# dusk-network/plonk

Hardware: NVIDIA H100
Metric: proofs/sec @ 2^16 gates (higher is better)
Workload: dtype u32 limbs (Fr 256-bit / Fp 384-bit Montgomery)

## Files before the change

### plonk_b200/csrc/msm.cu

```cuda
#include <algorithm>
#include <atomic>
#include <vector>

#include "common.cuh"
#include "g1.cuh"
#include "host_field.h"

struct pb200_srs {
  size_t n_points;
  int c;
  int W;
  uint4* table;
};

namespace pb {

static constexpr int kGroup = 8;
static constexpr unsigned kClassChunk = 512;
static constexpr unsigned kHeavyMin = 32, kHeavyFactor = 4;
static constexpr unsigned kHeavyChunk = 256;

PB_D G1Affine ld_affine(const uint4* p, size_t i) {
  const uint4* q = p + 6 * i;
  uint4 a0 = __ldg(q), a1 = __ldg(q + 1), a2 = __ldg(q + 2), b0 = __ldg(q + 3), b1 = __ldg(q + 4), b2 = __ldg(q + 5);
  G1Affine r;
  r.x.v[0] = a0.x; r.x.v[1] = a0.y; r.x.v[2] = a0.z; r.x.v[3] = a0.w;
  r.x.v[4] = a1.x; r.x.v[5] = a1.y; r.x.v[6] = a1.z; r.x.v[7] = a1.w;
  r.x.v[8] = a2.x; r.x.v[9] = a2.y; r.x.v[10] = a2.z; r.x.v[11] = a2.w;
  r.y.v[0] = b0.x; r.y.v[1] = b0.y; r.y.v[2] = b0.z; r.y.v[3] = b0.w;
  r.y.v[4] = b1.x; r.y.v[5] = b1.y; r.y.v[6] = b1.z; r.y.v[7] = b1.w;
  r.y.v[8] = b2.x; r.y.v[9] = b2.y; r.y.v[10] = b2.z; r.y.v[11] = b2.w;
  return r;
}
PB_D void st_fp(uint4* q, const Fp& f) {
  q[0] = make_uint4(f.v[0], f.v[1], f.v[2], f.v[3]);
  q[1] = make_uint4(f.v[4], f.v[5], f.v[6], f.v[7]);
  q[2] = make_uint4(f.v[8], f.v[9], f.v[10], f.v[11]);
}
PB_D Fp ld_fp(const uint4* q) {
  uint4 a = q[0], b = q[1], c = q[2];
  Fp f;
  f.v[0] = a.x; f.v[1] = a.y; f.v[2] = a.z; f.v[3] = a.w;
  f.v[4] = b.x; f.v[5] = b.y; f.v[6] = b.z; f.v[7] = b.w;
// ... 181 lines not shown
      val &= mask;
    }
    unsigned d = val + carry;
    unsigned sign = 0;
    if (d > half) {
      d = (1u << c) - d;
      sign = 1;
      carry = 1;
    } else {
      carry = 0;
    }
    const size_t slot = ((size_t)b * W + w) * n + i;
    if (d == 0) {
      ebkt[slot] = 0xffffffffu;
    } else {
      const unsigned bucket = d - 1;
      ebkt[slot] = (bucket << 1) | sign;
      epos[slot] = atomicAdd(&counts[(size_t)b * nb + bucket], 1u);
    }
  }
}

__global__ void __launch_bounds__(1024) k_msm_scan(const unsigned* counts, unsigned* offsets, unsigned* order, unsigned* n_heavy,
                                                   unsigned* heavy_pre, unsigned* max_len, unsigned nb, int size_shift) {
  __shared__ unsigned sums[1024];
  __shared__ unsigned bins[1024];
  __shared__ unsigned s_nh, s_total, s_thr_units, s_max;
  const unsigned b = blockIdx.x, tid = threadIdx.x;
  const unsigned* cnt = counts + (size_t)b * nb;
  unsigned* off = offsets + (size_t)b * (nb + 1);
  unsigned* ord = order + (size_t)b * nb;
  const unsigned chunk = (nb + 1023) / 1024;
  const unsigned lo = tid * chunk, hi = min(nb, lo + chunk);
  unsigned s = 0, mx = 0;
  for (unsigned k = lo; k < hi; k++) {
    s += cnt[k];
    mx = max(mx, cnt[k]);
  }
  sums[tid] = s;
  bins[tid] = 0;
  if (tid == 0) s_max = 0;
  __syncthreads();
  if (mx) atomicMax(&s_max, mx);
  for (unsigned d = 1; d < 1024; d <<= 1) {
    unsigned v = (tid >= d) ? sums[tid - d] : 0;
    __syncthreads();
    sums[tid] += v;
// ... 22 lines not shown
  }
  bins[tid] = sums[tid] - mine;
  if (tid == 0) {
    const unsigned avg = s_total / nb;
    const unsigned thr = max(kHeavyMin, kHeavyFactor * avg);
    s_thr_units = min(1021u, (thr + (1u << size_shift) - 1u) >> size_shift);
  }
  __syncthreads();
  if (tid == 1022u - s_thr_units) {
    n_heavy[b] = sums[tid];
    s_nh = sums[tid];
  }
  __syncthreads();
  for (unsigned k = tid; k < nb; k += 1024) {
    const unsigned pos = atomicAdd(&bins[1023u - min(cnt[k] >> size_shift, 1023u)], 1u);
    ord[pos] = k;
  }
  __syncthreads();
  const unsigned nh = s_nh;
  unsigned* hp = heavy_pre + (size_t)b * (nb + 1);
  const unsigned per = (nh + 1023u) / 1024u;
  const unsigned h_lo = min(nh, tid * per), h_hi = min(nh, h_lo + per);
  unsigned c = 0;
  for (unsigned h = h_lo; h < h_hi; h++) c += (cnt[ord[h]] + kHeavyChunk - 1) / kHeavyChunk;
  sums[tid] = c;
  __syncthreads();
  for (unsigned d = 1; d < 1024; d <<= 1) {
    unsigned v = (tid >= d) ? sums[tid - d] : 0;
    __syncthreads();
    sums[tid] += v;
    __syncthreads();
  }
  unsigned run2 = sums[tid] - c;
  for (unsigned h = h_lo; h < h_hi; h++) {
    hp[h] = run2;
    run2 += (cnt[ord[h]] + kHeavyChunk - 1) / kHeavyChunk;
  }
  if (tid == 1023) hp[nh] = sums[1023];
}

__global__ void k_msm_scatter(const unsigned* ebkt, const unsigned* epos, const unsigned* offsets, size_t n,
                              int W, unsigned nb, size_t n_table, size_t first, unsigned* sorted) {
  size_t i = (size_t)blockIdx.x * blockDim.x + threadIdx.x;
  if (i >= n) return;
  const unsigned w = blockIdx.y, b = blockIdx.z;
  const size_t slot = ((size_t)b * W + w) * n + i;
  const unsigned e = ebkt[slot];
  if (e == 0xffffffffu) return;
  const unsigned bucket = e >> 1, sign = e & 1u;
  const unsigned dst = offsets[(size_t)b * (nb + 1) + bucket] + epos[slot];
  sorted[(size_t)b * n * W + dst] = (unsigned)(((size_t)w * n_table + first + i) << 1) | sign;
}

PB_D G1Xyzz shfl_down_xyzz(const G1Xyzz& p, int delta, int width) {
  G1Xyzz r;
#pragma unroll
  for (int i = 0; i < 12; i++) {
    r.x.v[i] = __shfl_down_sync(0xffffffffu, p.x.v[i], delta, width);
    r.y.v[i] = __shfl_down_sync(0xffffffffu, p.y.v[i], delta, width);
// ... 38 lines not shown
      p_next = ld_affine(table, e_next >> 1);
    }
    if (p.is_inf()) continue;
    if (e & 1u) p.y = p.y.neg();
    xyzz_madd(acc, p.x, p.y);
  }
  for (int d = (int)split >> 1; d > 0; d >>= 1) {
    G1Xyzz o = shfl_down_xyzz(acc, d, (int)split);
    xyzz_add(acc, o);
  }
  if (valid && part == 0) st_xyzz(sums, (size_t)b * nb + bucket, acc);
}

PB_D G1Xyzz warp_sum(G1Xyzz v) {
  for (int d = 16; d > 0; d >>= 1) {
    G1Xyzz o = shfl_down_xyzz(v, d, 32);
    xyzz_add(v, o);
  }
  return v;
}

__global__ void __launch_bounds__(128) k_msm_heavy_chunks(const uint4* table, const unsigned* sorted, const unsigned* offsets,
                                                          const unsigned* order, const unsigned* n_heavy, const unsigned* heavy_pre,
                                                          unsigned nb, size_t cap, size_t part_cap, uint4* partials) {
  const unsigned b = blockIdx.y;
  const unsigned nh = n_heavy[b];
  if (nh == 0) return;
  const unsigned* hp = heavy_pre + (size_t)b * (nb + 1);
  const unsigned total = hp[nh];
  const unsigned* src = sorted + (size_t)b * cap;
  const unsigned* off = offsets + (size_t)b * (nb + 1);
  const unsigned* ord = order + (size_t)b * nb;
  const unsigned lane = threadIdx.x & 31, warps = gridDim.x * 4;
  for (unsigned v = blockIdx.x * 4 + (threadIdx.x >> 5); v < total; v += warps) {
    unsigned lo = 0, hi = nh;
    while (hi - lo > 1) {
      const unsigned mid = (lo + hi) >> 1;
      if (hp[mid] <= v) lo = mid; else hi = mid;
    }
    const unsigned bucket = ord[lo];
    const unsigned start = off[bucket] + (v - hp[lo]) * kHeavyChunk, end = min(off[bucket + 1], start + kHeavyChunk);
    G1Xyzz acc = G1Xyzz::identity();
    for (unsigned k = start + lane; k < end; k += 32) {
      const unsigned e = __ldg(src + k);
      G1Affine p = ld_affine(table, e >> 1);
      if (p.is_inf()) continue;
      if (e & 1u) p.y = p.y.neg();
      xyzz_madd(acc, p.x, p.y);
    }
    acc = warp_sum(acc);
    if (lane == 0) st_xyzz(partials, (size_t)b * part_cap + v, acc);
  }
}

__global__ void __launch_bounds__(128) k_msm_heavy_combine(const uint4* partials, const unsigned* order, const unsigned* n_heavy,
                                                           const unsigned* heavy_pre, unsigned nb, size_t part_cap, uint4* sums) {
  const unsigned b = blockIdx.y;
  const unsigned nh = n_heavy[b];
  const unsigned* hp = heavy_pre + (size_t)b * (nb + 1);
  const unsigned lane = threadIdx.x & 31, warps = gridDim.x * 4;
  for (unsigned h = blockIdx.x * 4 + (threadIdx.x >> 5); h < nh; h += warps) {
    G1Xyzz acc = G1Xyzz::identity();
    for (unsigned v = hp[h] + lane; v < hp[h + 1]; v += 32) {
      G1Xyzz q = ld_xyzz(partials, (size_t)b * part_cap + v);
// ... 344 lines not shown
  fetch(np - 1);
  Fp inv_run = ld_fp(a.ctot + 3 * ((size_t)b * a.ctas_max + blockIdx.x)) * ld_fp(a.factor + 3 * ((size_t)b * a.threads + t));
#pragma unroll 1
  for (int i = np - 1; i >= 0; i--) {
    const uint4 ds = a.desc[slot0 + (size_t)i * a.threads];
    asm volatile("cp.async.wait_group 0;" ::: "memory");
    G1Affine p1, p2;
    p1.x = ld_fp(stage); p1.y = ld_fp(stage + 3);
    p2.x = ld_fp(stage + 6); p2.y = ld_fp(stage + 9);
    const Fp pre = ld_fp(stage + 12);
    if (i > 0) fetch(i - 1);
    if (FIRST) {
      if ((ds.x & 1u) && !p1.is_inf()) p1.y = p1.y.neg();
      if ((ds.y & 1u) && !p2.is_inf()) p2.y = p2.y.neg();
    }
    Fp d = Fp::one();
    const int kind = aff_classify(p1, p2, &d);
    const Fp inv_d = inv_run * pre;
    inv_run = inv_run * d;
    aff_store(a, b, ds.z, aff_finish(kind, p1, p2, inv_d));
  }
}

struct DigitPlan {
  int ndig;
  int shift[8];
  int bits[8];
  int first_class[8];
  int n_digit_classes;
  int n_a_classes;
  int nclasses;
};

template <bool AFFINE>
__global__ void __launch_bounds__(64) k_msm_groups(const uint4* sums, unsigned nb, int g, uint4* S, uint4* A) {
  const unsigned G = blockIdx.x * blockDim.x + threadIdx.x;
  const unsigned n_groups = nb / g;
  if (G >= n_groups) return;
  const unsigned b = blockIdx.y;
  G1Xyzz run = G1Xyzz::identity(), acc = G1Xyzz::identity();
  for (int j = g - 1; j >= 0; j--) {
    if (AFFINE) {
      const G1Affine q = ld_affine(sums, (size_t)b * nb + (size_t)G * g + j);
      if (!q.is_inf()) xyzz_madd(run, q.x, q.y);
    } else {
      G1Xyzz q = ld_xyzz(sums, (size_t)b * nb + (size_t)G * g + j);
      xyzz_add(run, q);
    }
    xyzz_add(acc, run);
  }
  st_xyzz(S, (size_t)b * n_groups + G, run);
  st_xyzz(A, (size_t)b * n_groups + G, acc);
}

__global__ void __launch_bounds__(128) k_msm_group_classes(const uint4* S, const uint4* A, unsigned n_groups,
                                                           DigitPlan plan, unsigned chunks, uint4* out) {
  const int cls = blockIdx.x * 4 + (threadIdx.x >> 5);
  const int lane = threadIdx.x & 31;
  const unsigned b = blockIdx.y, chunk = blockIdx.z;
  if (cls >= plan.nclasses) return;
  G1Xyzz acc = G1Xyzz::identity();
  if (cls < plan.n_digit_classes) {
    int j = 0;
    while (j + 1 < plan.ndig && cls >= plan.first_class[j + 1]) j++;
    const unsigned v = cls - plan.first_class[j];
    const int sh_j = plan.shift[j], bits_j = plan.bits[j];
    const unsigned count = n_groups >> bits_j;
    for (unsigned idx = chunk * kClassChunk + lane; idx < min(count, (chunk + 1) * kClassChunk); idx += 32) {
      const unsigned G = ((idx >> sh_j) << (sh_j + bits_j)) | (v << sh_j) | (idx & ((1u << sh_j) - 1u));
      G1Xyzz q = ld_xyzz(S, (size_t)b * n_groups + G);
      xyzz_add(acc, q);
    }
  } else if (chunk == 0) {
    const unsigned first = (unsigned)(cls - plan.n_digit_classes) * 256u;
    for (unsigned G = first + lane; G < min(n_groups, first + 256u); G += 32) {
      G1Xyzz q = ld_xyzz(A, (size_t)b * n_groups + G);
      xyzz_add(acc, q);
    }
  }
  acc = warp_sum(acc);
  if (lane == 0) st_xyzz(out, ((size_t)b * plan.nclasses + cls) * chunks + chunk, acc);
}

__global__ void __launch_bounds__(256) k_msm_final(const uint4* classes, DigitPlan plan, unsigned chunks, uint4* out) {
  const int lane = threadIdx.x & 31, j = threadIdx.x >> 5;
  const unsigned b = blockIdx.x;
  if (j < plan.ndig) {
    const int nv = 1 << plan.bits[j];
    G1Xyzz x = G1Xyzz::identity();
    if (lane < nv)
      for (unsigned ch = 0; ch < chunks; ch++) {
        G1Xyzz q = ld_xyzz(classes, ((size_t)b * plan.nclasses + plan.first_class[j] + lane) * chunks + ch);
        xyzz_add(x, q);
      }
    for (int d = 1; d < nv; d <<= 1) {
      G1Xyzz o = shfl_down_xyzz(x, d, 32);
      if (lane + d < nv) xyzz_add(x, o);
    }
    G1Xyzz y = (lane >= 1 && lane < nv) ? x : G1Xyzz::identity();
    for (int d = nv >> 1; d > 0; d >>= 1) {
      G1Xyzz o = shfl_down_xyzz(y, d, 32);
      xyzz_add(y, o);
    }
    if (lane == 0) st_xyzz(out, (size_t)b * (plan.ndig + 1) + j, y);
  } else if (j == 7) {
    G1Xyzz acc = G1Xyzz::identity();
    for (int k = lane; k < plan.n_a_classes; k += 32) {
      G1Xyzz q = ld_xyzz(classes, ((size_t)b * plan.nclasses + plan.n_digit_classes + k) * chunks);
      xyzz_add(acc, q);
    }
    acc = warp_sum(acc);
    if (lane == 0) st_xyzz(out, (size_t)b * (plan.ndig + 1) + plan.ndig, acc);
  }
}

__global__ void k_selftest_fr_mul(const uint4* a, const uint4* b, uint4* o, size_t n) {
  size_t i = (size_t)blockIdx.x * blockDim.x + threadIdx.x;
  if (i >= n) return;
  Fr x, y;
  uint4 t0 = a[2 * i], t1 = a[2 * i + 1];
  x.v[0] = t0.x; x.v[1] = t0.y; x.v[2] = t0.z; x.v[3] = t0.w; x.v[4] = t1.x; x.v[5] = t1.y; x.v[6] = t1.z; x.v[7] = t1.w;
  t0 = b[2 * i]; t1 = b[2 * i + 1];
  y.v[0] = t0.x; y.v[1] = t0.y; y.v[2] = t0.z; y.v[3] = t0.w; y.v[4] = t1.x; y.v[5] = t1.y; y.v[6] = t1.z; y.v[7] = t1.w;
  Fr r = x * y;
  o[2 * i] = make_uint4(r.v[0], r.v[1], r.v[2], r.v[3]);
  o[2 * i + 1] = make_uint4(r.v[4], r.v[5], r.v[6], r.v[7]);
}
__global__ void k_selftest_fp_mul(const uint4* a, const uint4* b, uint4* o, size_t n) {
  size_t i = (size_t)blockIdx.x * blockDim.x + threadIdx.x;
  if (i >= n) return;
  Fp x = ld_fp(a + 3 * i), y = ld_fp(b + 3 * i);
  st_fp(o + 3 * i, x * y);
}

__global__ void k_selftest_fp_ops(const uint4* a, const uint4* b, const uint4* c, const uint4* d, uint4* o, size_t n) {
  size_t i = (size_t)blockIdx.x * blockDim.x + threadIdx.x;
// ... 39 lines not shown
std::atomic<int> g_prof_on{0};
std::atomic<uint64_t> g_prof_acc_ns{0}, g_prof_acc_adds{0}, g_prof_acc_launches{0}, g_prof_acc_points{0};
std::atomic<uint64_t> g_prof_sp_ns{0}, g_prof_sp_adds{0}, g_prof_sp_launches{0}, g_prof_sp_points{0};

static int pick_window(size_t n_points) {
  if (const char* env = getenv("PB200_MSM_C")) {
    int c = atoi(env);
    if (c >= 2 && c <= 20) return c;
  }
  int lg = 0;
  while (((size_t)1 << (lg + 1)) <= n_points) lg++;
  if (lg <= 16) return std::max(4, lg);
  return lg <= 19 ? 16 : 20;
}

static void xyzz_dev_to_host(const uint32_t* w, pbh::HXyzz* o) {
  memcpy(o->x.v, w, 48);
  memcpy(o->y.v, w + 12, 48);
  memcpy(o->zz.v, w + 24, 48);
  memcpy(o->zzz.v, w + 36, 48);
}

thread_local int t_msm_throughput_hint = 0;

struct MsmTail {
  DigitPlan plan;
  int log_g = 0;
  int c = 0;
  uint32_t batch = 0;
  size_t words_per_entry() const { return (size_t)(plan.ndig + 1) * 48; }
};

static bool msm_affine_enabled() {
  static const bool on = [] {
    const char* e = getenv("PB200_MSM_AFFINE");
    return e && atoi(e) != 0;
  }();
  return on;
}

static size_t aff_slots(size_t cap, size_t nb) {
  size_t widest = 0;
  for (int r = 0; ((size_t)1 << r) < cap || r == 0; r++) {
    const size_t positions = r == 0 ? cap : (cap >> r) + nb + 1;
    const size_t ctas = ((positions + kAffK - 1) / kAffK + kAffThreads - 1) / kAffThreads;
    widest = std::max(widest, ctas * kAffThreads);
// ... 2 lines not shown
}

static int msm_plan_c(int c, uint32_t batch, MsmTail* tail, unsigned* n_groups_out, int* g_out) {
  const unsigned nb = 1u << (c - 1);
  const int g = std::min<unsigned>(kGroup, nb);
  const unsigned n_groups = nb / g;
  int log_g = 0;
  while ((1 << log_g) < g) log_g++;
  DigitPlan& plan = tail->plan;
  int total_bits = 0;
  while ((1u << total_bits) < n_groups) total_bits++;
  plan.ndig = (total_bits + 3) / 4;
  if (plan.ndig > 7) return fail(PB200_ERR_INVALID_ARG, "window too wide for the bucket reduction");
  int sh = 0, cls = 0;
  for (int j = 0; j < plan.ndig; j++) {
    const int bits = (total_bits - sh) / (plan.ndig - j);
    plan.shift[j] = sh;
    plan.bits[j] = bits;
    plan.first_class[j] = cls;
    sh += bits;
    cls += 1 << bits;
  }
  plan.n_digit_classes = cls;
  plan.n_a_classes = (int)((n_groups + 255) / 256);
  plan.nclasses = plan.n_digit_classes + plan.n_a_classes;
  tail->log_g = log_g;
  tail->c = c;
  tail->batch = batch;
  *n_groups_out = n_groups;
  *g_out = g;
  return 0;
}
static int msm_plan(const pb200_srs* srs, uint32_t batch, MsmTail* tail, unsigned* n_groups_out, int* g_out) {
  return msm_plan_c(srs->c, batch, tail, n_groups_out, g_out);
}

static int msm_enqueue(const pb200_srs* srs, size_t first, const uint64_t* d_scalars, size_t n, uint32_t batch, size_t stride,
                       cudaStream_t st, ScratchScope& scope, uint4** d_result, MsmTail* tail, cudaEvent_t* prof_ev,
                       const unsigned** d_totals) {
  if (first + n > srs->n_points) return fail(PB200_ERR_DEGREE_TOO_LARGE, "more scalars than commit-key points");
  const int c = srs->c, W = srs->W;
  const unsigned nb = 1u << (c - 1);
  const size_t cap = n * (size_t)W;
  if (((srs->n_points * (size_t)W) << 1) >= ((size_t)1 << 32)) return fail(PB200_ERR_INVALID_ARG, "commit key too large for 32-bit point references");
  unsigned n_groups = 0;
  int g = 0;
  PB_TRY(msm_plan(srs, batch, tail, &n_groups, &g));
  const DigitPlan& plan = tail->plan;
  uint4* result = nullptr;
  PB_ALLOC(scope, result, (size_t)batch * (plan.ndig + 1) * 192);
  *d_result = result;
  if (n == 0) {
    PB_CUDA(cudaMemsetAsync(result, 0, (size_t)batch * (plan.ndig + 1) * 192, st));
    return 0;
  }

  int log_split = 0;
  if (!t_msm_throughput_hint) {
    const size_t avg = cap / nb;
    while (log_split < 5 && ((size_t)nb * batch << log_split) < (1u << 17) && (avg >> (log_split + 1)) >= 8) log_split++;
  }
  if (const char* env = getenv("PB200_MSM_LOG_SPLIT")) log_split = atoi(env);

  unsigned *counts = nullptr, *offsets = nullptr, *order = nullptr, *ebkt = nullptr, *epos = nullptr, *sorted = nullptr;
  uint4 *sums = nullptr, *classes = nullptr, *S = nullptr, *A = nullptr;
  PB_ALLOC(scope, counts, (size_t)batch * nb * 4);
  PB_ALLOC(scope, offsets, (size_t)batch * (nb + 1) * 4);
  PB_ALLOC(scope, order, (size_t)batch * nb * 4);
  const bool affine = msm_affine_enabled();
  unsigned *n_heavy = nullptr, *heavy_pre = nullptr, *max_len = nullptr;
  PB_ALLOC(scope, max_len, (size_t)batch * 4);
  PB_ALLOC(scope, n_heavy, (size_t)batch * 4);
  PB_ALLOC(scope, heavy_pre, (size_t)batch * (nb + 1) * 4);
  PB_ALLOC(scope, ebkt, (size_t)batch * cap * 4);
  PB_ALLOC(scope, epos, (size_t)batch * cap * 4);
  PB_ALLOC(scope, sorted, (size_t)batch * cap * 4);
  PB_ALLOC(scope, sums, (size_t)batch * nb * 192);
  unsigned chunks = 1;
  for (int j = 0; j < plan.ndig; j++) chunks = std::max<unsigned>(chunks, (unsigned)(((n_groups >> plan.bits[j]) + kClassChunk - 1) / kClassChunk));
  PB_ALLOC(scope, classes, (size_t)batch * plan.nclasses * chunks * 192);
  PB_ALLOC(scope, S, (size_t)batch * n_groups * 192);
  PB_ALLOC(scope, A, (size_t)batch * n_groups * 192);
  PB_CUDA(cudaMemsetAsync(counts, 0, (size_t)batch * nb * 4, st));

  PB_LAUNCH(k_msm_digits, dim3(div_up(n, 128), batch), 128, 0, st, (const uint4*)d_scalars, n, stride, c, W, nb,
            counts, ebkt, epos);
  int size_shift = 0;
  while (((cap / nb) >> size_shift) > 64) size_shift++;
  const size_t part_cap = cap / kHeavyChunk + std::min<size_t>(nb, cap / kHeavyMin) + 2;
  uint4* partials = nullptr;
  PB_ALLOC(scope, partials, (size_t)batch * part_cap * 192);
  PB_LAUNCH(k_msm_scan, batch, 1024, 0, st, counts, offsets, order, n_heavy, heavy_pre, max_len, nb, size_shift);
  PB_LAUNCH(k_msm_scatter, dim3(div_up(n, 256), W, batch), 256, 0, st, ebkt, epos, offsets, n, W, nb,
            srs->n_points, first, sorted);
  if (prof_ev) PB_CUDA(cudaEventRecord(prof_ev[0], st));
  if (affine) {
    const size_t capA = cap / 2 + nb + 2, capB = cap / 4 + nb + 2;
    int rounds = 0;
    while (((size_t)1 << rounds) < cap) rounds++;
    auto positions = [&](int r) { return r == 0 ? cap : (cap >> r) + nb + 1; };
    const size_t slots = aff_slots(cap, nb);
    uint4 *bufA = nullptr, *bufB = nullptr, *pre = nullptr, *factor = nullptr, *ctot = nullptr, *cpre = nullptr;
    uint4* desc = nullptr;
    unsigned* npairs = nullptr;
    const size_t threads_max = slots / (kAffK / 2);
    const unsigned ctas_max = (unsigned)(threads_max / kAffThreads);
    PB_ALLOC(scope, bufA, (size_t)batch * capA * 96);
    PB_ALLOC(scope, bufB, (size_t)batch * capB * 96);
    PB_ALLOC(scope, pre, (size_t)batch * slots * 48);
    PB_ALLOC(scope, desc, (size_t)batch * slots * 16);
    PB_ALLOC(scope, factor, (size_t)batch * threads_max * 48);
    PB_ALLOC(scope, npairs, (size_t)batch * threads_max * 4);
    PB_ALLOC(scope, ctot, (size_t)batch * ctas_max * 48);
    PB_ALLOC(scope, cpre, (size_t)batch * ctas_max * 48);
    PB_CUDA(cudaMemsetAsync(sums, 0, (size_t)batch * nb * 96, st));
// ... 2 lines not shown
      a.table = srs->table; a.sorted = sorted; a.offsets = offsets; a.max_len = max_len; a.prefix = pre; a.desc = desc; a.sums = sums;
      a.factor = factor; a.ctot = ctot; a.npairs = npairs; a.ctas_max = ctas_max;
      a.nb = nb; a.cap = cap; a.r = r;
      a.in = (r & 1) ? bufA : bufB;
      a.out = (r & 1) ? bufB : bufA;
      a.in_cap = (r & 1) ? capA : capB;
      a.out_cap = (r & 1) ? capB : capA;
      const unsigned ctas = div_up(div_up(positions(r), kAffK), kAffThreads);
      a.threads = ctas * kAffThreads;
      a.slots = slots;
      const size_t stage_bytes = (size_t)kAffThreads * 15 * 16;
      if (r == 0)
        PB_LAUNCH(k_msm_affine_fwd<true>, dim3(ctas, batch), kAffThreads, 0, st, a);
      else
        PB_LAUNCH(k_msm_affine_fwd<false>, dim3(ctas, batch), kAffThreads, 0, st, a);
      PB_LAUNCH(k_fp_batch_inverse, batch, 256, 0, st, ctot, cpre, ctas, (size_t)ctas_max, (const unsigned*)max_len, r);
      if (r == 0)
        PB_LAUNCH(k_msm_affine_back<true>, dim3(ctas, batch), kAffThreads, stage_bytes, st, a);
      else
        PB_LAUNCH(k_msm_affine_back<false>, dim3(ctas, batch), kAffThreads, stage_bytes, st, a);
    }
    if (prof_ev) PB_CUDA(cudaEventRecord(prof_ev[1], st));
    if (d_totals) *d_totals = offsets + nb;
    PB_LAUNCH(k_msm_groups<true>, dim3(div_up(n_groups, 64), batch), 64, 0, st, (const uint4*)sums, nb, g, S, A);
  } else {
  {
    static const int acc_block = [] {
      const char* e = getenv("PB200_ACC_BLOCK");
      return e ? atoi(e) : 128;
    }();
    if (acc_block == 64) {
      const dim3 grid(div_up((size_t)nb << log_split, 64), batch);
      PB_LAUNCH((k_msm_accumulate<64, 4>), grid, 64, 0, st, srs->table, sorted, offsets, order, n_heavy, nb, log_split, cap, sums);
    } else {
      const dim3 grid(div_up((size_t)nb << log_split, 128), batch);
      PB_LAUNCH((k_msm_accumulate<128, 2>), grid, 128, 0, st, srs->table, sorted, offsets, order, n_heavy, nb, log_split, cap, sums);
    }
  }
  if (d_totals) *d_totals = offsets + nb;
  PB_LAUNCH(k_msm_heavy_chunks, dim3(4 * num_sms(), batch), 128, 0, st, srs->table, sorted, offsets, order, n_heavy, heavy_pre, nb, cap, part_cap, partials);
  PB_LAUNCH(k_msm_heavy_combine, dim3(64, batch), 128, 0, st, (const uint4*)partials, order, n_heavy, heavy_pre, nb, part_cap, sums);
  if (prof_ev) PB_CUDA(cudaEventRecord(prof_ev[1], st));
    PB_LAUNCH(k_msm_groups<false>, dim3(div_up(n_groups, 64), batch), 64, 0, st, (const uint4*)sums, nb, g, S, A);
  }
  PB_LAUNCH(k_msm_group_classes, dim3(div_up(plan.nclasses, 4), batch, chunks), 128, 0, st, (const uint4*)S, (const uint4*)A,
            n_groups, plan, chunks, classes);
  PB_LAUNCH(k_msm_final, batch, 256, 0, st, (const uint4*)classes, plan, chunks, result);
  PB_CUDA(cudaGetLastError());
  return 0;
}

static void msm_finish(const uint32_t* host, const MsmTail& tail, int n_parts, uint64_t* out_affine_host) {
  const DigitPlan& plan = tail.plan;
  const uint32_t batch = tail.batch;
  const size_t wpe = tail.words_per_entry();
  std::vector<pbh::HXyzz> res(batch);
  for (uint32_t b = 0; b < batch; b++) {
    auto digit = [&](int d) {
      pbh::HXyzz s = pbh::HXyzz::identity(), t;
      for (int p = 0; p < n_parts; p++) {
        xyzz_dev_to_host(host + ((size_t)p * batch + b) * wpe + (size_t)d * 48, &t);
        pbh::hxyzz_add(s, t);
      }
      return s;
    };
    pbh::HXyzz h = pbh::HXyzz::identity();
    for (int d = plan.ndig - 1; d >= 0; d--) {
      pbh::HXyzz t = digit(d);
      pbh::hxyzz_add(h, t);
      const int dbl = d > 0 ? plan.bits[d - 1] : tail.log_g;
// ... 137 lines not shown
  scope.release();
  if (local_rc != 0) {
    g_last_error = local_msg;
    return local_rc;
  }
  std::vector<uint32_t> parts((size_t)n_ranks * payload / 4);
  for (int r = 0; r < n_ranks; r++) {
    const uint32_t* h = (const uint32_t*)(host + rec * (size_t)r);
    if (h[0] != 0) {
      char msg[48];
      snprintf(msg, sizeof msg, "rank %d", r);
      return fail(PB200_ERR_CUDA, "the partial MSM of another rank failed", msg);
    }
    if (h[1] != (uint32_t)tail.c || h[2] != (uint32_t)tail.plan.ndig || h[3] != batch)
      return fail(PB200_ERR_INVALID_ARG, "ranks disagree on the MSM window or batch (key slices must use one window width)");
    memcpy(parts.data() + (size_t)r * payload / 4, h + 4, payload);
  }
  msm_finish(parts.data(), tail, n_ranks, out_affine_host);
  return 0;
}

size_t msm_workspace_bytes(const pb200_srs* srs, size_t n, uint32_t batch) {
  const size_t nb = (size_t)1 << (srs->c - 1), cap = n * (size_t)srs->W;
  const size_t n_groups = std::max<size_t>(1, nb / kGroup);
  size_t b = 0;
  b += 4 * ((size_t)batch * (nb + 1) * 4 + 256);
  {
    int size_shift = 0;
    while (((cap / nb) >> size_shift) > 64) size_shift++;
    b += (size_t)batch * (cap / kHeavyChunk + std::min<size_t>(nb, cap / kHeavyMin) + 2) * 192 + 256;
  }
  b += (size_t)batch * 4 + 256;
  b += 3 * ((size_t)batch * cap * 4 + 256);
  b += (size_t)batch * nb * 192 + 256;
  b += 2 * ((size_t)batch * n_groups * 192 + 256);
  b += (size_t)batch * (8 * 16 + n_groups / 256 + 2) * (n_groups / (16 * kClassChunk) + 2) * 192 + 256;
  b += (size_t)batch * 9 * 192 + 256;
  if (msm_affine_enabled()) {
    b += (size_t)batch * ((cap / 2 + nb + 2) + (cap / 4 + nb + 2)) * 96 + 512;
    b += (size_t)batch * aff_slots(cap, nb) * (48 + 16) + 512;
    b += (size_t)batch * (aff_slots(cap, nb) / (kAffK / 2)) * (48 + 4 + 1) + 2048;
  }
  return b + 4096;
}

int srs_upload(const uint8_t* raw, size_t n_points, pb200_srs** out, int window_bits) {
  if (n_points == 0) return fail(PB200_ERR_INVALID_ARG, "empty commit key");
  cudaStream_t st = thread_stream();
  pb200_srs* s = new pb200_srs();
  s->n_points = n_points;
  s->c = window_bits ? window_bits : pick_window(n_points);
  s->W = (256 + s->c - 1) / s->c;
  s->table = nullptr;
  cudaError_t e = cudaMalloc((void**)&s->table, (size_t)s->W * n_points * 96);
  if (e != cudaSuccess) {
    delete s;
    return fail(PB200_ERR_CUDA, "cudaMalloc(commit key table)", cudaGetErrorString(e));
  }
  e = cudaMemcpyAsync(s->table, raw, n_points * 96, cudaMemcpyHostToDevice, st);
// ... 214 lines not shown
```

### plonk_b200/csrc/prover.cu

```cuda
#include <algorithm>
#include <mutex>
#include <vector>

#include "common.cuh"
#include "host_field.h"
#include "transcript.h"

struct pb200_srs;

namespace pb {

int ntt_run(const uint64_t* d_in, size_t in_len, uint64_t* d_out, uint32_t log_n, int inverse, int coset,
            uint32_t batch, size_t in_stride, size_t out_stride, cudaStream_t st, Arena* ar);
int msm_run(const pb200_srs* srs, size_t first, const uint64_t* d_scalars, size_t n, uint32_t batch,
            size_t stride, uint64_t* out_affine_host, cudaStream_t st, Arena* ar);
size_t msm_workspace_bytes(const pb200_srs* srs, size_t n, uint32_t batch);
int srs_upload(const uint8_t* raw, size_t n_points, pb200_srs** out);
void srs_free(pb200_srs* s);
size_t srs_len(const pb200_srs* s);
const uint4* srs_points(const pb200_srs* s);
int srs_from_device(const uint4* d_points, size_t n_points, pb200_srs** out, int window_bits);
int msm_window_for(size_t n_points);
extern thread_local int t_msm_throughput_hint;
static std::atomic<int> g_force_throughput{0};
int g1_check_raw(const uint8_t* raw, size_t n);
int raw_commit_key_parse(const uint8_t* bytes, size_t len, int checked, size_t* n_points, uint8_t* out_raw);
int lagrange_key_dev(const uint4* d_in, int log_n, uint4* d_out, cudaStream_t st);
int get_twiddles(int logm, bool inverse, cudaStream_t st, const uint4** out);
int fill_powers(uint4* out, size_t n, const Fr& base, const Fr& scale, cudaStream_t st);
Fr ntt_group_gen(int log_n, bool inverse);
Fr ntt_size_inv(int log_n);
Fr ntt_coset_gen(bool inverse);

enum { Q_M, Q_L, Q_R, Q_O, Q_F, Q_C, Q_ARITH, Q_RANGE, Q_LOGIC, Q_FIXED, Q_VAR, S1, S2, S3, S4, N_POLY };

PB_D Fr ldg_fr(const uint4* p, size_t i) {
  uint4 a = __ldg(p + 2 * i), b = __ldg(p + 2 * i + 1);
  Fr r;
  r.v[0] = a.x; r.v[1] = a.y; r.v[2] = a.z; r.v[3] = a.w;
  r.v[4] = b.x; r.v[5] = b.y; r.v[6] = b.z; r.v[7] = b.w;
  return r;
}
PB_D Fr ld_fr_plain(const uint4* p, size_t i) {
  uint4 a = p[2 * i], b = p[2 * i + 1];
  Fr r;
  r.v[0] = a.x; r.v[1] = a.y; r.v[2] = a.z; r.v[3] = a.w;
// ... 817 lines not shown
}

static pbh::Transcript base_transcript(const pb200_prover* P) {
  pbh::Transcript tr(P->label.data(), P->label.size());
  tr.circuit_domain_sep(P->constraints);
  static const char* lbl[N_POLY] = {"q_m", "q_l", "q_r", "q_o", "q_c", "q_f", "q_arith", "q_range", "q_logic",
                                    "q_variable_group_add", "q_fixed_group_add", "s_sigma_1", "s_sigma_2", "s_sigma_3", "s_sigma_4"};
  static const int ord[N_POLY] = {Q_M, Q_L, Q_R, Q_O, Q_C, Q_F, Q_ARITH, Q_RANGE, Q_LOGIC, Q_VAR, Q_FIXED, S1, S2, S3, S4};
  for (int i = 0; i < N_POLY; i++) tr.append_commitment(lbl[i], P->comm[ord[i]]);
  tr.circuit_domain_sep(P->constraints);
  return tr;
}

int prove_dev(const pb200_prover* P, const uint64_t* d_wit, const uint64_t* pi_idx, const uint64_t* pi_vals, size_t n_pi,
              const uint64_t* blinders_host, uint8_t* out_proof, cudaStream_t st) {
  const size_t n = P->n, n8 = P->n8, stride = n + 8;
  const int log_n = P->log_n;
  struct InFlight {
    const pb200_prover* P;
    explicit InFlight(const pb200_prover* p) : P(p) { P->active.fetch_add(1, std::memory_order_relaxed); }
    ~InFlight() {
      P->active.fetch_sub(1, std::memory_order_relaxed);
      t_msm_throughput_hint = 0;
    }
  } in_flight(P);
  static const int hint_at = [] {
    const char* e = getenv("PB200_THROUGHPUT_AT");
    return e ? atoi(e) : 2;
  }();
  const HFr* BL = (const HFr*)blinders_host;
  pbh::Transcript tr = base_transcript(P);
  const HFr* PIV = (const HFr*)pi_vals;
  if (n_pi && (!pi_idx || !pi_vals)) return fail(PB200_ERR_INVALID_ARG, "public inputs announced but not given");
  for (size_t i = 0; i < n_pi; i++) {
    if (pi_idx[i] >= P->constraints) return fail(PB200_ERR_INVALID_ARG, "public input index out of range");
    if (i && pi_idx[i] <= pi_idx[i - 1]) return fail(PB200_ERR_INVALID_ARG, "public input positions must be strictly increasing");
    tr.append_scalar("pi", PIV[i]);
  }
  const uint4* w_half = nullptr;
  PB_TRY(get_twiddles(log_n, false, st, &w_half));

  Arena arena;
  {
    std::lock_guard<std::mutex> lk(P->ws_mu);
    if (!P->ws_free.empty()) {
      arena = P->ws_free.back();
// ... 51 lines not shown
    for (size_t i = 0; i < n_pi; i++)
      PB_CUDA(cudaMemcpyAsync(pi_dense + 2 * pi_idx[i], PIV + i, 32, cudaMemcpyHostToDevice, st));
  }
  PB_CUDA(cudaMemsetAsync(zp, 0, 6 * stride * 32, st));
  PB_TRY(ntt_run((const uint64_t*)wv, n, (uint64_t*)wp, log_n, 1, 0, n_pi ? 5 : 4, n, stride, st, ar));
  {
    BlindArgs ba;
    ba.nb = 2;
    ba.npoly = 4;
    for (int p = 0; p < 4; p++)
      for (int i = 0; i < 2; i++) ba.b[p][i] = to_dev(BL[2 * p + i]);
    PB_LAUNCH(k_blind, 1, 32, 0, st, wp, stride, n, ba);
  }
  if (P->srs_lag) {
    uint4* sc = w8;
    PB_CUDA(cudaMemcpy2DAsync(sc, stride * 32, wv, n * 32, n * 32, 4, cudaMemcpyDeviceToDevice, st));
    BlindArgs ba;
    ba.nb = 2;
    ba.npoly = 4;
    for (int p = 0; p < 4; p++)
      for (int i = 0; i < 2; i++) ba.b[p][i] = to_dev(BL[2 * p + i]);
    PB_LAUNCH(k_lagrange_tail, 1, 32, 0, st, sc, stride, n, ba);
    t_msm_throughput_hint = 0;
    PB_TRY(msm_run(P->srs_lag, 0, (const uint64_t*)sc, n + 4, 4, stride, aff, st, ar));
  } else {
    t_msm_throughput_hint = (hint_at > 0 && (g_force_throughput.load(std::memory_order_relaxed) || P->active.load(std::memory_order_relaxed) >= hint_at)) ? 1 : 0;
    PB_TRY(msm_run(P->srs, 0, (const uint64_t*)wp, n + 2, 4, stride, aff, st, ar));
  }
  for (int k = 0; k < 4; k++) compress_affine(aff + 12 * k, c48[k]);
  tr.append_commitment("a_comm", c48[0]);
  tr.append_commitment("b_comm", c48[1]);
  tr.append_commitment("c_comm", c48[2]);
  tr.append_commitment("d_comm", c48[3]);

  const HFr beta = tr.challenge_scalar("beta");
  tr.append_scalar("beta", beta);
  const HFr gamma = tr.challenge_scalar("gamma");
  PB_LAUNCH(k_perm_terms, div_up(n, 128), 128, 0, st, (const uint4*)wv, (const uint4*)P->d_sigma, w_half, n, to_dev(beta), to_dev(gamma), num, den);
  PB_LAUNCH(k_batch_div, div_up(div_up(n, 8), 128), 128, 0, st, (const uint4*)num, (const uint4*)den, n, num);
  PB_TRY((fr_scan<true, false>(num, n, den, st, ar)));
  PB_TRY(ntt_run((const uint64_t*)den, n, (uint64_t*)zp, log_n, 1, 0, 1, n, stride, st, ar));
  {
    BlindArgs ba;
    ba.nb = 3;
    ba.npoly = 1;
    for (int i = 0; i < 3; i++) ba.b[0][i] = to_dev(BL[8 + i]);
    PB_LAUNCH(k_blind, 1, 32, 0, st, zp, stride, n, ba);
// ... 317 lines not shown
```

Before: 184.7.

## Restructure MSM bucket reduction into row/column sums and widen heavy chunks

Replaces the per-group running-sum (S,A) bucket reduction with a row/column decomposition. Row sums S feed the digit classes, and per-column partial sums P over runs of groups are combined in a weighted lane sum for the intra-group weights. An optional fold pass is added when there are many chunks, and the list chunk is smaller. Heavy-bucket chunk size becomes a runtime parameter and widens to 1024 under the throughput hint or a new thread-local flag set for the Lagrange-SRS path under concurrency. This exposes more parallelism and removes sequential running-sum work, at the cost of more kernels and a larger P buffer.

```diff
diff --git a/plonk_b200/csrc/msm.cu b/plonk_b200/csrc/msm.cu
--- a/plonk_b200/csrc/msm.cu
+++ b/plonk_b200/csrc/msm.cu
@@ -16,9 +16,8 @@
 namespace pb {
 
 static constexpr int kGroup = 8;
-static constexpr unsigned kClassChunk = 512;
 static constexpr unsigned kHeavyMin = 32, kHeavyFactor = 4;
-static constexpr unsigned kHeavyChunk = 256;
+static constexpr unsigned kHeavyChunk = 256, kHeavyChunkWide = 1024;
 
 PB_D G1Affine ld_affine(const uint4* p, size_t i) {
   const uint4* q = p + 6 * i;
@@ -246,7 +245,8 @@
 }
 
 __global__ void __launch_bounds__(1024) k_msm_scan(const unsigned* counts, unsigned* offsets, unsigned* order, unsigned* n_heavy,
-                                                   unsigned* heavy_pre, unsigned* max_len, unsigned nb, int size_shift) {
+                                                   unsigned* heavy_pre, unsigned* max_len, unsigned nb, int size_shift,
+                                                   unsigned heavy_chunk) {
   __shared__ unsigned sums[1024];
   __shared__ unsigned bins[1024];
   __shared__ unsigned s_nh, s_total, s_thr_units, s_max;
@@ -315,7 +315,7 @@
   const unsigned per = (nh + 1023u) / 1024u;
   const unsigned h_lo = min(nh, tid * per), h_hi = min(nh, h_lo + per);
   unsigned c = 0;
-  for (unsigned h = h_lo; h < h_hi; h++) c += (cnt[ord[h]] + kHeavyChunk - 1) / kHeavyChunk;
+  for (unsigned h = h_lo; h < h_hi; h++) c += (cnt[ord[h]] + heavy_chunk - 1) / heavy_chunk;
   sums[tid] = c;
   __syncthreads();
   for (unsigned d = 1; d < 1024; d <<= 1) {
@@ -327,7 +327,7 @@
   unsigned run2 = sums[tid] - c;
   for (unsigned h = h_lo; h < h_hi; h++) {
     hp[h] = run2;
-    run2 += (cnt[ord[h]] + kHeavyChunk - 1) / kHeavyChunk;
+    run2 += (cnt[ord[h]] + heavy_chunk - 1) / heavy_chunk;
   }
   if (tid == 1023) hp[nh] = sums[1023];
 }
@@ -412,7 +412,8 @@
 
 __global__ void __launch_bounds__(128) k_msm_heavy_chunks(const uint4* table, const unsigned* sorted, const unsigned* offsets,
                                                           const unsigned* order, const unsigned* n_heavy, const unsigned* heavy_pre,
-                                                          unsigned nb, size_t cap, size_t part_cap, uint4* partials) {
+                                                          unsigned nb, unsigned heavy_chunk, size_t cap, size_t part_cap,
+                                                          uint4* partials) {
   const unsigned b = blockIdx.y;
   const unsigned nh = n_heavy[b];
   if (nh == 0) return;
@@ -429,7 +430,7 @@
       if (hp[mid] <= v) lo = mid; else hi = mid;
     }
     const unsigned bucket = ord[lo];
-    const unsigned start = off[bucket] + (v - hp[lo]) * kHeavyChunk, end = min(off[bucket + 1], start + kHeavyChunk);
+    const unsigned start = off[bucket] + (v - hp[lo]) * heavy_chunk, end = min(off[bucket + 1], start + heavy_chunk);
     G1Xyzz acc = G1Xyzz::identity();
     for (unsigned k = start + lane; k < end; k += 32) {
       const unsigned e = __ldg(src + k);
@@ -820,96 +821,107 @@
   }
 }
 
+static constexpr unsigned kColRun = 8;
+static constexpr unsigned kListChunk = 256;
+static constexpr unsigned kFinalChunks = 4;
+
 struct DigitPlan {
   int ndig;
   int shift[8];
   int bits[8];
   int first_class[8];
   int n_digit_classes;
-  int n_a_classes;
-  int nclasses;
+  int n_columns;
+  int nlists;
 };
 
 template <bool AFFINE>
-__global__ void __launch_bounds__(64) k_msm_groups(const uint4* sums, unsigned nb, int g, uint4* S, uint4* A) {
-  const unsigned G = blockIdx.x * blockDim.x + threadIdx.x;
-  const unsigned n_groups = nb / g;
-  if (G >= n_groups) return;
+PB_D void add_bucket(G1Xyzz& acc, const uint4* sums, size_t i) {
+  if (AFFINE) {
+    const G1Affine q = ld_affine(sums, i);
+    if (!q.is_inf()) xyzz_madd(acc, q.x, q.y);
+  } else {
+    xyzz_add(acc, ld_xyzz(sums, i));
+  }
+}
+
+template <bool AFFINE>
+__global__ void __launch_bounds__(64) k_msm_rows_cols(const uint4* sums, unsigned nb, unsigned g, unsigned col_run, uint4* S, uint4* P) {
+  const unsigned t = blockIdx.x * blockDim.x + threadIdx.x;
+  const unsigned n_groups = nb / g, n_parts = n_groups / col_run;
   const unsigned b = blockIdx.y;
-  G1Xyzz run = G1Xyzz::identity(), acc = G1Xyzz::identity();
-  for (int j = g - 1; j >= 0; j--) {
-    if (AFFINE) {
-      const G1Affine q = ld_affine(sums, (size_t)b * nb + (size_t)G * g + j);
-      if (!q.is_inf()) xyzz_madd(run, q.x, q.y);
-    } else {
-      G1Xyzz q = ld_xyzz(sums, (size_t)b * nb + (size_t)G * g + j);
-      xyzz_add(run, q);
-    }
-    xyzz_add(acc, run);
-  }
-  st_xyzz(S, (size_t)b * n_groups + G, run);
-  st_xyzz(A, (size_t)b * n_groups + G, acc);
-}
-
-__global__ void __launch_bounds__(128) k_msm_group_classes(const uint4* S, const uint4* A, unsigned n_groups,
-                                                           DigitPlan plan, unsigned chunks, uint4* out) {
-  const int cls = blockIdx.x * 4 + (threadIdx.x >> 5);
+  const size_t base = (size_t)b * nb;
+  G1Xyzz acc = G1Xyzz::identity();
+  if (t < n_groups) {
+    for (unsigned j = 0; j < g; j++) add_bucket<AFFINE>(acc, sums, base + (size_t)t * g + j);
+    st_xyzz(S, (size_t)b * n_groups + t, acc);
+  } else if (t < n_groups + g * n_parts) {
+    const unsigned u = t - n_groups, j = u / n_parts, part = u % n_parts;
+    for (unsigned k = 0; k < col_run; k++) add_bucket<AFFINE>(acc, sums, base + (size_t)(part * col_run + k) * g + j);
+    st_xyzz(P, ((size_t)b * g + j) * n_parts + part, acc);
+  }
+}
+
+__global__ void __launch_bounds__(128) k_msm_lists(const uint4* S, const uint4* P, unsigned n_groups, unsigned n_parts,
+                                                   DigitPlan plan, unsigned chunks, uint4* out) {
+  const int list = blockIdx.x * 4 + (threadIdx.x >> 5);
   const int lane = threadIdx.x & 31;
   const unsigned b = blockIdx.y, chunk = blockIdx.z;
-  if (cls >= plan.nclasses) return;
+  if (list >= plan.nlists) return;
   G1Xyzz acc = G1Xyzz::identity();
-  if (cls < plan.n_digit_classes) {
+  if (list < plan.n_digit_classes) {
     int j = 0;
-    while (j + 1 < plan.ndig && cls >= plan.first_class[j + 1]) j++;
-    const unsigned v = cls - plan.first_class[j];
+    while (j + 1 < plan.ndig && list >= plan.first_class[j + 1]) j++;
+    const unsigned v = list - plan.first_class[j];
     const int sh_j = plan.shift[j], bits_j = plan.bits[j];
     const unsigned count = n_groups >> bits_j;
-    for (unsigned idx = chunk * kClassChunk + lane; idx < min(count, (chunk + 1) * kClassChunk); idx += 32) {
+    for (unsigned idx = chunk * kListChunk + lane; idx < min(count, (chunk + 1) * kListChunk); idx += 32) {
       const unsigned G = ((idx >> sh_j) << (sh_j + bits_j)) | (v << sh_j) | (idx & ((1u << sh_j) - 1u));
-      G1Xyzz q = ld_xyzz(S, (size_t)b * n_groups + G);
-      xyzz_add(acc, q);
-    }
-  } else if (chunk == 0) {
-    const unsigned first = (unsigned)(cls - plan.n_digit_classes) * 256u;
-    for (unsigned G = first + lane; G < min(n_groups, first + 256u); G += 32) {
-      G1Xyzz q = ld_xyzz(A, (size_t)b * n_groups + G);
-      xyzz_add(acc, q);
-    }
+      xyzz_add(acc, ld_xyzz(S, (size_t)b * n_groups + G));
+    }
+  } else {
+    const size_t col = (size_t)b * plan.n_columns + (list - plan.n_digit_classes);
+    for (unsigned idx = chunk * kListChunk + lane; idx < min(n_parts, (chunk + 1) * kListChunk); idx += 32)
+      xyzz_add(acc, ld_xyzz(P, col * n_parts + idx));
   }
   acc = warp_sum(acc);
-  if (lane == 0) st_xyzz(out, ((size_t)b * plan.nclasses + cls) * chunks + chunk, acc);
-}
-
-__global__ void __launch_bounds__(256) k_msm_final(const uint4* classes, DigitPlan plan, unsigned chunks, uint4* out) {
-  const int lane = threadIdx.x & 31, j = threadIdx.x >> 5;
+  if (lane == 0) st_xyzz(out, ((size_t)b * plan.nlists + list) * chunks + chunk, acc);
+}
+
+__global__ void __launch_bounds__(128) k_msm_fold(const uint4* in, unsigned n_sets, unsigned chunks, uint4* out) {
+  const unsigned set = blockIdx.x * 4 + (threadIdx.x >> 5), lane = threadIdx.x & 31;
+  if (set >= n_sets) return;
+  G1Xyzz acc = G1Xyzz::identity();
+  for (unsigned k = lane; k < chunks; k += 32) xyzz_add(acc, ld_xyzz(in, (size_t)set * chunks + k));
+  acc = warp_sum(acc);
+  if (lane == 0) st_xyzz(out, set, acc);
+}
+
+PB_D G1Xyzz weighted_lane_sum(G1Xyzz x, int lane, int n, int first) {
+  for (int d = 1; d < n; d <<= 1) {
+    G1Xyzz o = shfl_down_xyzz(x, d, 32);
+    if (lane + d < n) xyzz_add(x, o);
+  }
+  G1Xyzz y = (lane >= first && lane < n) ? x : G1Xyzz::identity();
+  for (int d = n >> 1; d > 0; d >>= 1) {
+    G1Xyzz o = shfl_down_xyzz(y, d, 32);
+    xyzz_add(y, o);
+  }
+  return y;
+}
+
+__global__ void __launch_bounds__(256) k_msm_final(const uint4* lists, DigitPlan plan, unsigned chunks, uint4* out) {
+  const int lane = threadIdx.x & 31, w = threadIdx.x >> 5;
   const unsigned b = blockIdx.x;
-  if (j < plan.ndig) {
-    const int nv = 1 << plan.bits[j];
-    G1Xyzz x = G1Xyzz::identity();
-    if (lane < nv)
-      for (unsigned ch = 0; ch < chunks; ch++) {
-        G1Xyzz q = ld_xyzz(classes, ((size_t)b * plan.nclasses + plan.first_class[j] + lane) * chunks + ch);
-        xyzz_add(x, q);
-      }
-    for (int d = 1; d < nv; d <<= 1) {
-      G1Xyzz o = shfl_down_xyzz(x, d, 32);
-      if (lane + d < nv) xyzz_add(x, o);
-    }
-    G1Xyzz y = (lane >= 1 && lane < nv) ? x : G1Xyzz::identity();
-    for (int d = nv >> 1; d > 0; d >>= 1) {
-      G1Xyzz o = shfl_down_xyzz(y, d, 32);
-      xyzz_add(y, o);
-    }
-    if (lane == 0) st_xyzz(out, (size_t)b * (plan.ndig + 1) + j, y);
-  } else if (j == 7) {
-    G1Xyzz acc = G1Xyzz::identity();
-    for (int k = lane; k < plan.n_a_classes; k += 32) {
-      G1Xyzz q = ld_xyzz(classes, ((size_t)b * plan.nclasses + plan.n_digit_classes + k) * chunks);
-      xyzz_add(acc, q);
-    }
-    acc = warp_sum(acc);
-    if (lane == 0) st_xyzz(out, (size_t)b * (plan.ndig + 1) + plan.ndig, acc);
-  }
+  if (w >= plan.ndig && w != 7) return;
+  const bool digit = w < plan.ndig;
+  const int n = digit ? 1 << plan.bits[w] : plan.n_columns;
+  const int first_list = digit ? plan.first_class[w] : plan.n_digit_classes;
+  G1Xyzz x = G1Xyzz::identity();
+  if (lane < n)
+    for (unsigned ch = 0; ch < chunks; ch++) xyzz_add(x, ld_xyzz(lists, ((size_t)b * plan.nlists + first_list + lane) * chunks + ch));
+  const G1Xyzz y = weighted_lane_sum(x, lane, n, digit ? 1 : 0);
+  if (lane == 0) st_xyzz(out, (size_t)b * (plan.ndig + 1) + (digit ? w : plan.ndig), y);
 }
 
 __global__ void k_selftest_fr_mul(const uint4* a, const uint4* b, uint4* o, size_t n) {
@@ -995,6 +1007,7 @@
 }
 
 thread_local int t_msm_throughput_hint = 0;
+thread_local int t_msm_wide_heavy_chunks = 0;
 
 struct MsmTail {
   DigitPlan plan;
@@ -1043,8 +1056,8 @@
     cls += 1 << bits;
   }
   plan.n_digit_classes = cls;
-  plan.n_a_classes = (int)((n_groups + 255) / 256);
-  plan.nclasses = plan.n_digit_classes + plan.n_a_classes;
+  plan.n_columns = g;
+  plan.nlists = plan.n_digit_classes + plan.n_columns;
   tail->log_g = log_g;
   tail->c = c;
   tail->batch = batch;
@@ -1054,6 +1067,12 @@
 }
 static int msm_plan(const pb200_srs* srs, uint32_t batch, MsmTail* tail, unsigned* n_groups_out, int* g_out) {
   return msm_plan_c(srs->c, batch, tail, n_groups_out, g_out);
+}
+
+static unsigned reduction_chunks(const DigitPlan& plan, unsigned n_groups, unsigned n_parts) {
+  unsigned chunks = (n_parts + kListChunk - 1) / kListChunk;
+  for (int j = 0; j < plan.ndig; j++) chunks = std::max(chunks, ((n_groups >> plan.bits[j]) + kListChunk - 1) / kListChunk);
+  return std::max(chunks, 1u);
 }
 
 static int msm_enqueue(const pb200_srs* srs, size_t first, const uint64_t* d_scalars, size_t n, uint32_t batch, size_t stride,
@@ -1084,7 +1103,7 @@
   if (const char* env = getenv("PB200_MSM_LOG_SPLIT")) log_split = atoi(env);
 
   unsigned *counts = nullptr, *offsets = nullptr, *order = nullptr, *ebkt = nullptr, *epos = nullptr, *sorted = nullptr;
-  uint4 *sums = nullptr, *classes = nullptr, *S = nullptr, *A = nullptr;
+  uint4 *sums = nullptr, *lists = nullptr, *S = nullptr, *P = nullptr;
   PB_ALLOC(scope, counts, (size_t)batch * nb * 4);
   PB_ALLOC(scope, offsets, (size_t)batch * (nb + 1) * 4);
   PB_ALLOC(scope, order, (size_t)batch * nb * 4);
@@ -1097,21 +1116,22 @@
   PB_ALLOC(scope, epos, (size_t)batch * cap * 4);
   PB_ALLOC(scope, sorted, (size_t)batch * cap * 4);
   PB_ALLOC(scope, sums, (size_t)batch * nb * 192);
-  unsigned chunks = 1;
-  for (int j = 0; j < plan.ndig; j++) chunks = std::max<unsigned>(chunks, (unsigned)(((n_groups >> plan.bits[j]) + kClassChunk - 1) / kClassChunk));
-  PB_ALLOC(scope, classes, (size_t)batch * plan.nclasses * chunks * 192);
+  const unsigned col_run = std::min(kColRun, n_groups), n_parts = n_groups / col_run;
+  const unsigned chunks = reduction_chunks(plan, n_groups, n_parts);
+  PB_ALLOC(scope, lists, (size_t)batch * plan.nlists * chunks * 192);
   PB_ALLOC(scope, S, (size_t)batch * n_groups * 192);
-  PB_ALLOC(scope, A, (size_t)batch * n_groups * 192);
+  PB_ALLOC(scope, P, (size_t)batch * g * n_parts * 192);
   PB_CUDA(cudaMemsetAsync(counts, 0, (size_t)batch * nb * 4, st));
 
   PB_LAUNCH(k_msm_digits, dim3(div_up(n, 128), batch), 128, 0, st, (const uint4*)d_scalars, n, stride, c, W, nb,
             counts, ebkt, epos);
   int size_shift = 0;
   while (((cap / nb) >> size_shift) > 64) size_shift++;
+  const unsigned heavy_chunk = (t_msm_throughput_hint || t_msm_wide_heavy_chunks) ? kHeavyChunkWide : kHeavyChunk;
   const size_t part_cap = cap / kHeavyChunk + std::min<size_t>(nb, cap / kHeavyMin) + 2;
   uint4* partials = nullptr;
   PB_ALLOC(scope, partials, (size_t)batch * part_cap * 192);
-  PB_LAUNCH(k_msm_scan, batch, 1024, 0, st, counts, offsets, order, n_heavy, heavy_pre, max_len, nb, size_shift);
+  PB_LAUNCH(k_msm_scan, batch, 1024, 0, st, counts, offsets, order, n_heavy, heavy_pre, max_len, nb, size_shift, heavy_chunk);
   PB_LAUNCH(k_msm_scatter, dim3(div_up(n, 256), W, batch), 256, 0, st, ebkt, epos, offsets, n, W, nb,
             srs->n_points, first, sorted);
   if (prof_ev) PB_CUDA(cudaEventRecord(prof_ev[0], st));
@@ -1160,7 +1180,7 @@
     }
     if (prof_ev) PB_CUDA(cudaEventRecord(prof_ev[1], st));
     if (d_totals) *d_totals = offsets + nb;
-    PB_LAUNCH(k_msm_groups<true>, dim3(div_up(n_groups, 64), batch), 64, 0, st, (const uint4*)sums, nb, g, S, A);
+    PB_LAUNCH(k_msm_rows_cols<true>, dim3(div_up(n_groups + g * n_parts, 64), batch), 64, 0, st, (const uint4*)sums, nb, (unsigned)g, col_run, S, P);
   } else {
   {
     static const int acc_block = [] {
@@ -1176,14 +1196,20 @@
     }
   }
   if (d_totals) *d_totals = offsets + nb;
-  PB_LAUNCH(k_msm_heavy_chunks, dim3(4 * num_sms(), batch), 128, 0, st, srs->table, sorted, offsets, order, n_heavy, heavy_pre, nb, cap, part_cap, partials);
+  PB_LAUNCH(k_msm_heavy_chunks, dim3(4 * num_sms(), batch), 128, 0, st, srs->table, sorted, offsets, order, n_heavy, heavy_pre, nb, heavy_chunk, cap,
+            part_cap, partials);
   PB_LAUNCH(k_msm_heavy_combine, dim3(64, batch), 128, 0, st, (const uint4*)partials, order, n_heavy, heavy_pre, nb, part_cap, sums);
   if (prof_ev) PB_CUDA(cudaEventRecord(prof_ev[1], st));
-    PB_LAUNCH(k_msm_groups<false>, dim3(div_up(n_groups, 64), batch), 64, 0, st, (const uint4*)sums, nb, g, S, A);
-  }
-  PB_LAUNCH(k_msm_group_classes, dim3(div_up(plan.nclasses, 4), batch, chunks), 128, 0, st, (const uint4*)S, (const uint4*)A,
-            n_groups, plan, chunks, classes);
-  PB_LAUNCH(k_msm_final, batch, 256, 0, st, (const uint4*)classes, plan, chunks, result);
+    PB_LAUNCH(k_msm_rows_cols<false>, dim3(div_up(n_groups + g * n_parts, 64), batch), 64, 0, st, (const uint4*)sums, nb, (unsigned)g, col_run, S, P);
+  }
+  PB_LAUNCH(k_msm_lists, dim3(div_up(plan.nlists, 4), batch, chunks), 128, 0, st, (const uint4*)S, (const uint4*)P, n_groups, n_parts, plan,
+            chunks, lists);
+  if (chunks > kFinalChunks) {
+    PB_LAUNCH(k_msm_fold, div_up((size_t)batch * plan.nlists, 4), 128, 0, st, (const uint4*)lists, batch * (unsigned)plan.nlists, chunks, S);
+    PB_LAUNCH(k_msm_final, batch, 256, 0, st, (const uint4*)S, plan, 1u, result);
+  } else {
+    PB_LAUNCH(k_msm_final, batch, 256, 0, st, (const uint4*)lists, plan, chunks, result);
+  }
   PB_CUDA(cudaGetLastError());
   return 0;
 }
@@ -1367,7 +1393,11 @@
 
 size_t msm_workspace_bytes(const pb200_srs* srs, size_t n, uint32_t batch) {
   const size_t nb = (size_t)1 << (srs->c - 1), cap = n * (size_t)srs->W;
-  const size_t n_groups = std::max<size_t>(1, nb / kGroup);
+  MsmTail tail;
+  unsigned n_groups = 0;
+  int g = 0;
+  if (msm_plan(srs, batch, &tail, &n_groups, &g) != 0) return 0;
+  const unsigned n_parts = n_groups / std::min(kColRun, n_groups);
   size_t b = 0;
   b += 4 * ((size_t)batch * (nb + 1) * 4 + 256);
   {
@@ -1378,8 +1408,9 @@
   b += (size_t)batch * 4 + 256;
   b += 3 * ((size_t)batch * cap * 4 + 256);
   b += (size_t)batch * nb * 192 + 256;
-  b += 2 * ((size_t)batch * n_groups * 192 + 256);
-  b += (size_t)batch * (8 * 16 + n_groups / 256 + 2) * (n_groups / (16 * kClassChunk) + 2) * 192 + 256;
+  b += (size_t)batch * n_groups * 192 + 256;
+  b += (size_t)batch * g * n_parts * 192 + 256;
+  b += (size_t)batch * tail.plan.nlists * reduction_chunks(tail.plan, n_groups, n_parts) * 192 + 256;
   b += (size_t)batch * 9 * 192 + 256;
   if (msm_affine_enabled()) {
     b += (size_t)batch * ((cap / 2 + nb + 2) + (cap / 4 + nb + 2)) * 96 + 512;
diff --git a/plonk_b200/csrc/prover.cu b/plonk_b200/csrc/prover.cu
--- a/plonk_b200/csrc/prover.cu
+++ b/plonk_b200/csrc/prover.cu
@@ -22,6 +22,7 @@
 int srs_from_device(const uint4* d_points, size_t n_points, pb200_srs** out, int window_bits);
 int msm_window_for(size_t n_points);
 extern thread_local int t_msm_throughput_hint;
+extern thread_local int t_msm_wide_heavy_chunks;
 static std::atomic<int> g_force_throughput{0};
 int g1_check_raw(const uint8_t* raw, size_t n);
 int raw_commit_key_parse(const uint8_t* bytes, size_t len, int checked, size_t* n_points, uint8_t* out_raw);
@@ -885,6 +886,7 @@
     ~InFlight() {
       P->active.fetch_sub(1, std::memory_order_relaxed);
       t_msm_throughput_hint = 0;
+      t_msm_wide_heavy_chunks = 0;
     }
   } in_flight(P);
   static const int hint_at = [] {
@@ -982,7 +984,9 @@
       for (int i = 0; i < 2; i++) ba.b[p][i] = to_dev(BL[2 * p + i]);
     PB_LAUNCH(k_lagrange_tail, 1, 32, 0, st, sc, stride, n, ba);
     t_msm_throughput_hint = 0;
+    t_msm_wide_heavy_chunks = (hint_at > 0 && (g_force_throughput.load(std::memory_order_relaxed) || P->active.load(std::memory_order_relaxed) >= hint_at)) ? 1 : 0;
     PB_TRY(msm_run(P->srs_lag, 0, (const uint64_t*)sc, n + 4, 4, stride, aff, st, ar));
+    t_msm_wide_heavy_chunks = 0;
   } else {
     t_msm_throughput_hint = (hint_at > 0 && (g_force_throughput.load(std::memory_order_relaxed) || P->active.load(std::memory_order_relaxed) >= hint_at)) ? 1 : 0;
     PB_TRY(msm_run(P->srs, 0, (const uint64_t*)wp, n + 2, 4, stride, aff, st, ar));
```

New measurement: 190.6, median of 6. 3.2% higher.
